# haoheliu/voicefixer

Measured on AMD Instinct MI355X. Metric: seconds-of-44.1kHz-audio restored per wall-second, higher is better.
Workload: dtype f32

## Files before the change

### voicefixer_amd/csrc/vfx_conv.hip

```cpp
#include "vfx_common.h"
#include <cstdio>
#include <cstdlib>
#include <cstring>
#include <map>
#include <mutex>
#include <string>
#include <type_traits>
#include <vector>

#ifndef VFX_X3_ABL
#define VFX_X3_ABL 0
#endif
#ifndef VFX_ABL
#define VFX_ABL 0
#endif
#define VFX_MAXPH 8
#define VFX_MAXT 9

typedef float f32x16 __attribute__((ext_vector_type(16)));
typedef unsigned int u32x4 __attribute__((ext_vector_type(4)));

#if VFX_ABL & 8
__device__ unsigned long long g_dbg[10];
__device__ unsigned long long g_dbgx[6];
extern "C" int vfx_debug_read(unsigned long long* out, int reset) {
    hipMemcpyFromSymbol(out, HIP_SYMBOL(g_dbg), sizeof(unsigned long long) * 10);
    if (reset) { unsigned long long z[10] = {0}; hipMemcpyToSymbol(HIP_SYMBOL(g_dbg), z, sizeof(z)); }
    return 0;
}
extern "C" int vfx_debug_read_x(unsigned long long* out, int reset) {
    hipMemcpyFromSymbol(out, HIP_SYMBOL(g_dbgx), sizeof(unsigned long long) * 6);
    if (reset) { unsigned long long z[6] = {0}; hipMemcpyToSymbol(HIP_SYMBOL(g_dbgx), z, sizeof(z)); }
    return 0;
}
__device__ unsigned long long* g_trace_buf;
__device__ unsigned int g_trace_cap, g_trace_n;
extern "C" int vfx_debug_trace(unsigned long long* buf, unsigned int cap_records) {
    const unsigned int z = 0;
    hipMemcpyToSymbol(HIP_SYMBOL(g_trace_buf), &buf, sizeof(buf));
    hipMemcpyToSymbol(HIP_SYMBOL(g_trace_cap), &cap_records, sizeof(cap_records));
    hipMemcpyToSymbol(HIP_SYMBOL(g_trace_n), &z, sizeof(z));
    return 0;
}
extern "C" unsigned int vfx_debug_trace_count(void) {
    unsigned int n = 0;
    hipMemcpyFromSymbol(&n, HIP_SYMBOL(g_trace_n), sizeof(n));
    return n;
}
#define DBG_T(v) const unsigned long long v = __builtin_amdgcn_s_memtime()
#else
#define DBG_T(v)
#endif

struct PhaseTab {
    int ntaps, nseg, ooff, pad_;
    int seg_org[VFX_MAXT];
    int tap_lds[VFX_MAXT];
    int tap_w[VFX_MAXT];
};
struct ConvTables {
    PhaseTab ph[VFX_MAXPH];
};

struct ConvArgs {
    const float* x;
    const float* w;
    const float* bias;
    const float* res;
    float* y;
    const float* pre_scale;
    const float* pre_shift;
    const ConvTables* tab;
    int B, Cin, CinPad, Cout, Lin, Lq, Lout;
    long long x_bs, x_cs, y_bs, y_cs, y_ls, r_bs, r_cs, r_ls;
    int segw;
    int xs_floats;
    int ws_floats;
    int q_shift, q_mask, o_rs, o_cs;
    int pad_mode, pre_act, post_act;
    float pre_slope, post_slope;
    int in_mask, out_mask;
    int tile_lo, tile_hi;
    int tpw;
    int x_guard;
    int ksplit, cpp, ws_ls;
    float* ws;
    int bl_step;
    int nxv;
    int two_level;
    int res_init;
    const void* w3;
    const ConvTables* tab3;
    int segw3;
    int xplane3;
    int buf3;
    int bl3;
    int xrow3, wrow3;
    const float* wd;
    int kcx;
    int ntiles_l, xcd_chunk;
    int nph_fold;
    int wg_d;
    const int* x_rows;
    int lq_extra;
    int stagger, stagger_wgs;
    int w_tap0, w_tapstep, w_slab0, w_slabstep, w_slab_ph, w_ooff0, w_ooff_ph, w_nseg, w_seg0, w_segstep;
    const float* wd2;
    const float* bias2;
    int yp;
    float mid_slope;
    int rb_nq1;
    int rs_pshift, rs_nseg;
};

template <int KC>
struct StageCfg {
    static constexpr int MAXXV = 4;
    static constexpr int MAXWV = KC == 16 ? 6 : (KC == 8 ? 4 : 5);
};

template <int MAXXV, int MAXWV>
struct StageState {
    int x_l[MAXXV];
    int x_kc[MAXXV];
    int x_off[MAXXV];
    int w_off[MAXWV];
    float4 xv[MAXXV];
    float4 wv[MAXWV];
};

template <bool FAST, int MAXXV, int MAXWV>
__device__ __forceinline__ void stage_load(StageState<MAXXV, MAXWV>& st, const ConvArgs& a,
                                           const float* __restrict__ xb, int xcs, int c0, int lshift,
                                           __amdgpu_buffer_rsrc_t xrsrc, __amdgpu_buffer_rsrc_t wrsrc, int Lin_row) {
    if constexpr (FAST) {
        const int xso = (c0 * xcs + lshift) * 4, wso = c0 * a.Cout * 4;
#pragma unroll
        for (int j = 0; j < MAXXV; ++j) {
            const u32x4 r = __builtin_amdgcn_raw_buffer_load_b128(xrsrc, st.x_off[j], xso, 0);
            st.xv[j] = make_float4(__uint_as_float(r.x), __uint_as_float(r.y), __uint_as_float(r.z), __uint_as_float(r.w));
        }
#pragma unroll
        for (int j = 0; j < MAXWV; ++j) {
            const u32x4 r = __builtin_amdgcn_raw_buffer_load_b128(wrsrc, st.w_off[j], wso, 0);
            st.wv[j] = make_float4(__uint_as_float(r.x), __uint_as_float(r.y), __uint_as_float(r.z), __uint_as_float(r.w));
        }
        return;
    }
    const float* __restrict__ xc = xb + (long long)c0 * xcs + lshift;
    const float* __restrict__ wc = a.w + (long long)c0 * a.Cout;
#pragma unroll
    for (int j = 0; j < MAXXV; ++j) {
        if constexpr (FAST) {
            st.xv[j] = *reinterpret_cast<const float4*>(xc + st.x_off[j]);
        } else {
            const int Lin = Lin_row;
            const bool reflect = a.pad_mode == VFX_PAD_REFLECT;
            float4 v = make_float4(0.f, 0.f, 0.f, 0.f);
            const int kc = st.x_kc[j];
            if (c0 + kc < a.Cin) {
                const float* row = xc + (long long)kc * xcs;
                const int l = st.x_l[j];
                if (l >= 0 && l + 3 < Lin) {
                    v = *reinterpret_cast<const float4*>(row + l);
                } else {
                    float e[4];
#pragma unroll
                    for (int k = 0; k < 4; ++k) {
                        int g = l + k;
                        if (reflect) {
                            if (g < 0) g = -g;
                            if (g >= Lin) g = 2 * (Lin - 1) - g;
                        }
                        e[k] = (g >= 0 && g < Lin) ? row[g] : 0.f;
                    }
                    v = make_float4(e[0], e[1], e[2], e[3]);
                }
            }
            st.xv[j] = v;
        }
    }
#pragma unroll
    for (int j = 0; j < MAXWV; ++j) st.wv[j] = *reinterpret_cast<const float4*>(wc + st.w_off[j]);
}

template <int NTHR, int MAXXV, int MAXWV>
__device__ __forceinline__ void stage_write_plain(StageState<MAXXV, MAXWV>& st, const ConvArgs& a, float* xs, float* ws,
                                                  int nxv, int nwv, int xtotal, int wtotal, int tid) {
    const float slope = a.pre_act == VFX_PRE_LRELU ? a.pre_slope : 1.f;
#pragma unroll
    for (int j = 0; j < MAXXV; ++j) {
        if (j < nxv) {
            float4 v = st.xv[j];
            v.x = v.x > 0.f ? v.x : v.x * slope;
            v.y = v.y > 0.f ? v.y : v.y * slope;
            v.z = v.z > 0.f ? v.z : v.z * slope;
            v.w = v.w > 0.f ? v.w : v.w * slope;
            int i = tid + NTHR * j;
            i = i < xtotal ? i : xtotal - 1;
            *reinterpret_cast<float4*>(xs + 4 * i) = v;
        }
    }
#pragma unroll
    for (int j = 0; j < MAXWV; ++j)
        if (j < nwv) {
            int i = tid + NTHR * j;
            i = i < wtotal ? i : wtotal - 1;
            *reinterpret_cast<float4*>(ws + 4 * i) = st.wv[j];
        }
}

template <bool FAST, int NTHR, int MAXXV, int MAXWV>
__device__ __forceinline__ void stage_write(StageState<MAXXV, MAXWV>& st, const ConvArgs& a, int c0, float* xs,
                                            float* ws, const float* aff, int nxv, int nwv, int xtotal,
                                            int wtotal, int tid, int lshift, bool range_mask, int Lin_row) {
    const int pre_act = a.pre_act;
    const float pre_slope = a.pre_slope;
    const int in_mask = a.in_mask;
#pragma unroll
    for (int j = 0; j < MAXXV; ++j) {
        if (j < nxv) {
            float e[4] = {st.xv[j].x, st.xv[j].y, st.xv[j].z, st.xv[j].w};
            if (pre_act == VFX_PRE_LRELU) {
#pragma unroll
                for (int k = 0; k < 4; ++k) e[k] = vfx_lrelu(e[k], pre_slope);
            } else if (pre_act == VFX_PRE_AFFINE_LRELU) {
                const int c = c0 + st.x_kc[j];
                const float sc = aff[2 * c], sh = aff[2 * c + 1];
#pragma unroll
                for (int k = 0; k < 4; ++k) e[k] = vfx_lrelu(fmaf(e[k], sc, sh), pre_slope);
                if constexpr (!FAST) {
                    const int l = st.x_l[j] + lshift;
                    const bool cbad = c >= a.Cin;
                    if (a.pad_mode != VFX_PAD_REFLECT) {
#pragma unroll
                        for (int k = 0; k < 4; ++k)
                            if (l + k < 0 || l + k >= Lin_row || cbad) e[k] = 0.f;
                    }
                }
            }
            if constexpr (FAST) {
                if (range_mask) {
                    const int l = st.x_l[j] + lshift;
#pragma unroll
                    for (int k = 0; k < 4; ++k)
                        if (l + k < 0 || l + k >= Lin_row) e[k] = 0.f;
                }
            }
            if (in_mask >= 3) {
                const int l = st.x_l[j] + lshift;
                if (((l + 3) & in_mask) == in_mask) e[3] = 0.f;
            } else if (in_mask) {
                const int l = st.x_l[j] + lshift;
#pragma unroll
                for (int k = 0; k < 4; ++k)
                    if (((l + k) & in_mask) == in_mask) e[k] = 0.f;
            }
            int i = tid + NTHR * j;
            i = i < xtotal ? i : xtotal - 1;
            *reinterpret_cast<float4*>(xs + 4 * i) = make_float4(e[0], e[1], e[2], e[3]);
        }
    }
#pragma unroll
    for (int j = 0; j < MAXWV; ++j)
        if (j < nwv) {
// ... 1081 lines not shown
        const float quant = (float)nwg / (float)(((nwg + slots - 1) / slots) * slots);
        const float score = t.util * tail * quant;
        if (score > best_score * 1.02f) { best_score = score; best = i; }
    }
    if (best < 0) return VFX_EINVAL;
    const TileCfg& tc = kTiles[best];

    static const bool waves8_env = VFX_DEV_ENV("VFX_WAVES8") && atoi(VFX_DEV_ENV("VFX_WAVES8")) != 0;
    const bool waves8 = waves8_env && ((tc.BM == 128 && tc.BL == 128) || (tc.BM == 64 && tc.BL == 256));
    const int nthr = waves8 ? 512 : 256;
    static const bool kc16_env = VFX_DEV_ENV("VFX_KC16") && atoi(VFX_DEV_ENV("VFX_KC16")) != 0;
    int maxspan = 0;
    bool all_segments = true;
    for (int p = 0; p < nphase; ++p) {
        int mn = phs[p].taps[0].off, mx = mn;
        for (int t = 1; t < phs[p].ntaps; ++t) {
            mn = phs[p].taps[t].off < mn ? phs[p].taps[t].off : mn;
            mx = phs[p].taps[t].off > mx ? phs[p].taps[t].off : mx;
        }
        maxspan = mx - mn > maxspan ? mx - mn : maxspan;
        all_segments &= !((long long)tc.BL + (mx - mn) + 3 <= (long long)phs[p].ntaps * (tc.BL + 3));
    }
    static const int exact_off = VFX_DEV_ENV("VFX_NO_EXACT") ? atoi(VFX_DEV_ENV("VFX_NO_EXACT")) : 0;
    bool exact = exact_off != 1 && x->guard > 0 && pad_mode != VFX_PAD_REFLECT && in_mask == 0 && !waves8 &&
                 ((maxspan > 0 && maxspan <= 8) || (all_segments && exact_off != 2));
    ConvTables tb;
    int KC, ntiles;
    size_t lds;
    for (;;) {
        KC = (kc16_env && maxnt <= 3 && tc.BM == 128 && tc.BL == 128 && !waves8 && Cin % 16 == 0) ? 16 : 8;
        for (;;) {
            std::memset(&tb, 0, sizeof(tb));
            int rc = fill_segments(a, tb, nphase, phs, tc.BL, KC, exact);
            if (rc) return rc;
            int maxseg = 0;
            for (int p = 0; p < nphase; ++p) maxseg = tb.ph[p].nseg > maxseg ? tb.ph[p].nseg : maxseg;
            const bool xfit = (long long)maxseg * KC * (a.segw / 4) <= 4 * nthr;
            a.nxv = (int)(((long long)maxseg * KC * (a.segw / 4) + nthr - 1) / nthr);
            const bool wfit = (long long)maxnt * KC * tc.BM <= (KC == 16 ? 6 : (KC == 8 ? 4 : 5)) * 4 * nthr;
            if (xfit && wfit) break;
            if (KC == 4) return VFX_ERANGE;
            KC = KC == 16 ? 8 : 4;
        }
        a.ws_floats = maxnt * KC * tc.BM;
        lds = (2ull * (a.xs_floats + a.ws_floats) + 2ull * a.CinPad) * sizeof(float);
        {
            static const long pad_kb = VFX_DEV_ENV("VFX_LDS_MIN_KB") ? atol(VFX_DEV_ENV("VFX_LDS_MIN_KB")) : 0;
            if (pad_kb > 0 && lds < (size_t)pad_kb * 1024) lds = (size_t)pad_kb * 1024;
        }
        if (lds > 160 * 1024) return VFX_ERANGE;

        a.bl_step = (exact && !all_segments) ? tc.BL - maxspan : tc.BL;
        ntiles = (Lq + a.bl_step - 1) / a.bl_step;
        int seg_lo = 0x7fffffff, seg_hi = -0x7fffffff;
        for (int p = 0; p < nphase; ++p)
            for (int sg = 0; sg < tb.ph[p].nseg; ++sg) {
                seg_lo = tb.ph[p].seg_org[sg] < seg_lo ? tb.ph[p].seg_org[sg] : seg_lo;
                seg_hi = tb.ph[p].seg_org[sg] > seg_hi ? tb.ph[p].seg_org[sg] : seg_hi;
            }
        const long long g = (x->guard > 0 && pad_mode != VFX_PAD_REFLECT) ? x->guard : 0;
        const long long need_lo = -(long long)seg_lo - g;
        int tlo = need_lo > 0 ? (int)((need_lo + a.bl_step - 1) / a.bl_step) : 0;
        const long long room = (long long)Lin + g - seg_hi - a.segw;
        int thi = room >= 0 ? (int)(room / a.bl_step) + 1 : 0;
        if (thi > ntiles) thi = ntiles;
        if (tlo > thi || Cin % KC != 0) { tlo = 0; thi = 0; }
        if (((long long)a.CinPad * x->cstride + Lin + 2 * g) * 4 >= (1ll << 31) - (1ll << 20)) { tlo = 0; thi = 0; }
        if (a.x_rows && pad_mode == VFX_PAD_REFLECT) { tlo = 0; thi = 0; }
        a.tile_lo = tlo;
        a.tile_hi = thi;
        if (exact && !(tlo == 0 && thi == ntiles)) { exact = false; continue; }
        break;
    }
    a.tab = device_tables(tb);
    if (!a.tab) return VFX_EINVAL;
    a.two_level = KC == 4 && Cin >= 256;
    g_last_tile = tc.BM * 100000 + tc.BL * 100 + KC;
    a.ksplit = 1;
    {
        static const bool splitk_off = VFX_DEV_ENV("VFX_NO_SPLITK") && atoi(VFX_DEV_ENV("VFX_NO_SPLITK")) != 0;
        const int nchunks = (Cin + KC - 1) / KC;
        const long long nwg = (long long)ntiles * (nphase * Cout / tc.BM) * B;
        const bool plain_map = nphase == 1 && q_shift == 31 && o_rs == 0 && o_cs == 1 && phs[0].ooff == 0 && Lq <= Lout;
        if (!splitk_off && plain_map && nwg <= 192 && nchunks >= 32) {
            int want = (int)(512 / nwg);
            if (want > 8) want = 8;
            if (want > nchunks / 16) want = nchunks / 16;
            if (want >= 2 && (long long)B * want <= 65535) {
                a.cpp = (nchunks + want - 1) / want;
                a.ksplit = (nchunks + a.cpp - 1) / a.cpp;
                a.ws_ls = Lq;
                a.ws = splitk_workspace(stream, (size_t)a.ksplit * B * Cout * Lq * sizeof(float));
                if (!a.ws) a.ksplit = 1;
            }
        }
    }
    {
        const long long nwg1 = (long long)(a.tile_hi - a.tile_lo) * (nphase * Cout / tc.BM) * B;
        (void)nwg1;
        a.tpw = 1;
    }
    const int gy = nphase * Cout / tc.BM;
    const int gz = B * a.ksplit;
    int rc = VFX_EINVAL;
    if (KC == 16) rc = launch_cfg<128, 128, 2, 2, 16>(a, ntiles, gy, gz, lds, stream);
#define VFX_CASE(BM_, BL_, WGM_, WGL_)                                                          \
    else if (tc.BM == BM_ && tc.BL == BL_)                                                      \
        rc = KC == 8 ? launch_cfg<BM_, BL_, WGM_, WGL_, 8>(a, ntiles, gy, gz, lds, stream)      \
                     : launch_cfg<BM_, BL_, WGM_, WGL_, 4>(a, ntiles, gy, gz, lds, stream);
    else if (waves8 && tc.BM == 128 && tc.BL == 128)
        rc = KC == 8 ? launch_cfg<128, 128, 4, 2, 8>(a, ntiles, gy, gz, lds, stream)
                     : launch_cfg<128, 128, 4, 2, 4>(a, ntiles, gy, gz, lds, stream);
    else if (waves8 && tc.BM == 64 && tc.BL == 256)
        rc = KC == 8 ? launch_cfg<64, 256, 2, 4, 8>(a, ntiles, gy, gz, lds, stream)
                     : launch_cfg<64, 256, 2, 4, 4>(a, ntiles, gy, gz, lds, stream);
    VFX_CASE(128, 128, 2, 2)
    VFX_CASE(64, 256, 1, 4)
    VFX_CASE(128, 64, 4, 1)
    VFX_CASE(32, 256, 1, 4)
    VFX_CASE(64, 64, 2, 2)
    VFX_CASE(32, 128, 1, 4)
#undef VFX_CASE
    if (rc != VFX_OK || a.ksplit == 1) return rc;
    const long long total = (long long)B * Cout * Lq;
    const int blocks = (int)((total + 255) / 256 < 4096 ? (total + 255) / 256 : 4096);
    hipLaunchKernelGGL(splitk_reduce_kernel, dim3(blocks), dim3(256), 0, stream, a.ws, a.ksplit, a.ws_ls, a.bias, a.res,
                       a.r_bs, a.r_cs, a.r_ls, a.y, a.y_bs, a.y_cs, a.y_ls, B, Cout, Lq, a.post_act, a.post_slope,
                       a.out_mask);
    VFX_LAUNCHED();
    return vfx_last_error();
}

extern "C" int vfx_conv1d_f32(const vfx_tensor* x, const float* w_packed, const float* bias,
                              const vfx_tensor* res, const vfx_tensor* y, int B, int Cin, int Cout,
                              int L, int k, int dilation, int pad_mode, const vfx_act* act,
                              vfx_stream_t stream) {
    if (k < 1 || k > VFX_MAXT || !(k & 1) || dilation < 1) return VFX_EINVAL;
    PhaseSpec ph;
    ph.ntaps = k;
    ph.ooff = 0;
    for (int t = 0; t < k; ++t) {
        ph.taps[t].off = (t - (k - 1) / 2) * dilation;
        ph.taps[t].slab = t;
    }
    return launch_conv(x, w_packed, bias, res, y, B, Cin, Cout, L, L, L, 1, &ph, 31, 0x7fffffff, 0, 1,
                       pad_mode, act, 0, 0, (hipStream_t)stream);
}

extern "C" int vfx_convtr1d_f32(const vfx_tensor* x, const float* w_packed, const float* bias,
                                const vfx_tensor* y, int B, int Cin, int Cout, int Lin, int stride,
                                const vfx_act* act, vfx_stream_t stream) {
    if (stride < 1 || stride > VFX_MAXPH) return VFX_EINVAL;
    if (act && act->w_wino4) {
        const int rc = try_launch_convtw(x, act->w_wino4, bias, y, B, Cin, Cout, Lin, stride, act, (hipStream_t)stream);
        if (rc != VFX_ENOTSUP) return rc;
    }
    const int pad = stride / 2 + stride % 2;
    PhaseSpec ph[VFX_MAXPH];
    for (int r = 0; r < stride; ++r) {
        ph[r].ntaps = 2;
        ph[r].taps[0].off = 0;
        ph[r].taps[0].slab = r;
        ph[r].taps[1].off = -1;
        ph[r].taps[1].slab = r + stride;
        ph[r].ooff = r - pad;
    }
    return launch_conv(x, w_packed, bias, nullptr, y, B, Cin, Cout, Lin, Lin + 1, stride * Lin, stride, ph,
                       31, 0x7fffffff, 0, stride, VFX_PAD_ZERO, act, 0, 0, (hipStream_t)stream);
}

extern "C" int vfx_conv2d_f32(const vfx_tensor* x, const float* w_packed, const float* bias,
                              const vfx_tensor* res, const vfx_tensor* y, int B, int Cin, int Cout, int H,
                              int pitch_log2, int ksize, const vfx_act* act, vfx_stream_t stream) {
    if ((ksize != 1 && ksize != 3) || pitch_log2 < 1 || pitch_log2 > 12 || H < 1) return VFX_EINVAL;
    const int P = 1 << pitch_log2;
    PhaseSpec ph;
    ph.ooff = 0;
    ph.ntaps = ksize * ksize;
    for (int ky = 0; ky < ksize; ++ky)
        for (int kx = 0; kx < ksize; ++kx) {
            ph.taps[ky * ksize + kx].off = (ky - ksize / 2) * P + (kx - ksize / 2);
            ph.taps[ky * ksize + kx].slab = ky * ksize + kx;
        }
    const int L = H * P;
    return launch_conv(x, w_packed, bias, res, y, B, Cin, Cout, L, L, L, 1, &ph, 31, 0x7fffffff, 0, 1,
                       VFX_PAD_ZERO, act, P - 1, P - 1, (hipStream_t)stream);
}

extern "C" int vfx_convtr2d_3x3s2_f32(const vfx_tensor* x, const float* w_packed, const vfx_tensor* y, int B,
                                      int Cin, int Cout, int h, int in_pitch_log2, const vfx_act* act,
                                      vfx_stream_t stream) {
    if (in_pitch_log2 < 1 || in_pitch_log2 > 11 || h < 1) return VFX_EINVAL;
    const int Pi = 1 << in_pitch_log2, Po = 2 * Pi;
    PhaseSpec ph[4];
    for (int py = 0; py < 2; ++py)
        for (int px = 0; px < 2; ++px) {
            PhaseSpec& p = ph[py * 2 + px];
            p.ntaps = 0;
            p.ooff = py * Po + px;
            const int nky = py == 0 ? 2 : 1, nkx = px == 0 ? 2 : 1;
            for (int iy = 0; iy < nky; ++iy)
                for (int ix = 0; ix < nkx; ++ix) {
                    const int ky = py == 0 ? 2 * iy : 1, kx = px == 0 ? 2 * ix : 1;
                    const int dy = py == 0 ? iy : 0, dx = px == 0 ? ix : 0;
                    p.taps[p.ntaps].off = -(dy * Pi + dx);
                    p.taps[p.ntaps].slab = ky * 3 + kx;
                    ++p.ntaps;
                }
        }
    const int Lin = h * Pi;
    return launch_conv(x, w_packed, nullptr, nullptr, y, B, Cin, Cout, Lin, Lin, 2 * h * Po, 4, ph,
                       in_pitch_log2, Pi - 1, 2 * Po, 2, VFX_PAD_ZERO, act, Pi - 1, Po - 1,
                       (hipStream_t)stream);
}
```

### voicefixer_amd/csrc/vfx_convtw.inc

```
template <int WGM, int WGP>
__global__ __launch_bounds__(256, 2) void convtw_kernel(const ConvArgs a) {
    static_assert(WGM * WGP == 4, "four waves");
    constexpr int KC = 16, NSTEP = KC / 2, NPL = 4;
    constexpr int BM = 32 * WGM, BT = 32 * WGP;
    constexpr int CG = 256 / BT;
    constexpr int NSLOT = KC / CG;
    constexpr int SPAN = NSTEP / NSLOT;
    constexpr int PLANE = KC * BT;
    constexpr int BUF = NPL * PLANE;
    extern __shared__ __attribute__((aligned(16))) float smem[];

    const int tid = threadIdx.x, lane = tid & 63;
    const int wave = __builtin_amdgcn_readfirstlane(tid >> 6);
    const int lo = lane & 31, hi = lane >> 5;
    const int wm = wave / WGP, wp = wave % WGP;
    const int s = a.nph_fold, gy = a.tpw;
    int lin = blockIdx.x;
    if (a.xcd_chunk > 0) lin = (lin & 7) * a.xcd_chunk + (lin >> 3);
    if (lin >= a.ntiles_l * s * gy) return;
    int phase, mblk, tile;
    if (a.tile_lo == 0) {
        tile = lin % a.ntiles_l;
        const int rest = lin / a.ntiles_l;
        phase = rest % s; mblk = rest / s;
    } else {
        phase = lin % s;
        const int rest = lin / s;
        mblk = rest % gy; tile = rest / gy;
    }
    const int b = blockIdx.z;
    const int Lrow = a.x_rows ? __builtin_amdgcn_readfirstlane(a.x_rows[b]) : a.Lin;
    const int T0 = tile * BT;
    if (3 * T0 > Lrow) return;
    const int xcs = (int)a.x_cs;
    const int S = a.Cin / KC;

    const int st = tid % BT, cg = tid / BT;
    int xvoff[4];
    {
        const int p0 = 3 * (T0 + st) - 1;
#pragma unroll
        for (int j = 0; j < 4; ++j) xvoff[j] = (p0 + j >= 0 && p0 + j < Lrow) ? (cg * xcs + p0 + j) * 4 : VFX_W_OOB;
    }
    const __amdgpu_buffer_rsrc_t xrsrc = __builtin_amdgcn_make_buffer_rsrc(
        const_cast<float*>(a.x) + (long long)b * a.x_bs, (short)0, 0x7fffffff, 0x00020000);
    float* const wbase = smem + cg * BT + st;
    float xv[NSLOT][4];
    auto x_load_part = [&](int j, int t, int s0) {
        xv[j][t] = __uint_as_float(__builtin_amdgcn_raw_buffer_load_b32(xrsrc, xvoff[t], s0 + j * CG * xcs * 4, 0));
    };
    auto x_load = [&](int chunk) {
        const int s0 = chunk * KC * xcs * 4;
#pragma unroll
        for (int j = 0; j < NSLOT; ++j)
#pragma unroll
            for (int t = 0; t < 4; ++t) x_load_part(j, t, s0);
    };
    auto x_transform = [&](int j, float (&V)[4]) {
        V[0] = xv[j][0] - xv[j][2];
        V[1] = xv[j][1] + xv[j][2];
        V[2] = xv[j][2] - xv[j][1];
        V[3] = xv[j][3] - xv[j][1];
    };

    const __amdgpu_buffer_rsrc_t wrsrc =
        __builtin_amdgcn_make_buffer_rsrc(const_cast<float*>(a.wd), (short)0, 0x7fffffff, 0x00020000);
    const int row0 = mblk * BM + wm * 32;
    const int avoff = ((row0 + lo) * 8 + 4 * hi) * 4;
    const int gstride = a.Cout * 32;
    const int pstride = (a.CinPad >> 3) * gstride;
    const int poff = phase * NPL * pstride;
    float4 aw[2][NPL];
    auto a_load_one = [&](auto set_tag, int k, int grp) {
        constexpr int SET = decltype(set_tag)::value;
        const u32x4 r = __builtin_amdgcn_raw_buffer_load_b128(wrsrc, avoff, poff + k * pstride + grp * gstride, 0);
        aw[SET][k] = make_float4(__uint_as_float(r.x), __uint_as_float(r.y), __uint_as_float(r.z), __uint_as_float(r.w));
    };
    using S0 = std::integral_constant<int, 0>;
    using S1 = std::integral_constant<int, 1>;

    const __amdgpu_buffer_rsrc_t brsrc = __builtin_amdgcn_make_buffer_rsrc(
        const_cast<float*>(a.bias ? a.bias : a.x), (short)0, 0x7fffffff, 0x00020000);
    u32x4 bq[4];
    {
        const int bvoff = a.bias ? (row0 + 4 * hi) * 4 : VFX_W_OOB;
#pragma unroll
        for (int g = 0; g < 4; ++g) bq[g] = __builtin_amdgcn_raw_buffer_load_b128(brsrc, bvoff, g * 32, 0);
    }
    x_load(0);
#pragma unroll
    for (int k = 0; k < NPL; ++k) a_load_one(S0{}, k, 0);
    __builtin_amdgcn_sched_barrier(0);

    f32x16 acc[NPL];
    const int boffs = hi * BT + wp * 32 + lo;
    f32x16 biasv;
#pragma unroll
    for (int g = 0; g < 4; ++g) {
        biasv[4 * g + 0] = __uint_as_float(bq[g].x); biasv[4 * g + 1] = __uint_as_float(bq[g].y);
        biasv[4 * g + 2] = __uint_as_float(bq[g].z); biasv[4 * g + 3] = __uint_as_float(bq[g].w);
    }
    auto mma_chunk = [&](auto first_tag, const float* xs, float* wdst, int xchunk, int agrp0) {
        constexpr bool FIRST = decltype(first_tag)::value;
        const float* bp = xs + boffs;
        const int agrp1 = min(agrp0 + 1, 2 * S - 1), agrp2 = min(agrp0 + 2, 2 * S - 1);
        float bf[NPL];
#pragma unroll
        for (int k = 0; k < NPL; ++k) bf[k] = bp[k * PLANE];
        const int xs0 = xchunk * KC * xcs * 4;
        float V[4];
#pragma unroll
        for (int u = 0; u < NSTEP; ++u) {
            const int el = u / SPAN, ph = u % SPAN;
#pragma unroll
            for (int k = 0; k < NPL; ++k) {
                if (ph == 0 && k == 0) x_transform(el, V);
                if (ph == 0) wdst[el * CG * BT + k * PLANE] = V[k];
                if (ph == SPAN / 2) x_load_part(el, k, xs0);
                if (u == 0) a_load_one(S1{}, k, agrp1);
                if (u == 4) a_load_one(S0{}, k, agrp2);
                const float4 av4 = (u < 4) ? aw[0][k] : aw[1][k];
                const int kk = u & 3;
                const float av = kk == 0 ? av4.x : (kk == 1 ? av4.y : (kk == 2 ? av4.z : av4.w));
                if (FIRST && u == 0) {
                    const f32x16 zero16 = {0.f, 0.f, 0.f, 0.f, 0.f, 0.f, 0.f, 0.f, 0.f, 0.f, 0.f, 0.f, 0.f, 0.f, 0.f, 0.f};
                    acc[k] = __builtin_amdgcn_mfma_f32_32x32x2f32(av, bf[k], k == 1 ? biasv : zero16, 0, 0, 0);
                } else {
                    acc[k] = __builtin_amdgcn_mfma_f32_32x32x2f32(av, bf[k], acc[k], 0, 0, 0);
                }
                if (u < NSTEP - 1) bf[k] = bp[k * PLANE + (u + 1) * 2 * BT];
                __builtin_amdgcn_sched_barrier(0);
            }
        }
    };
    {
#pragma unroll
        for (int j = 0; j < NSLOT; ++j) {
            float V[4];
            x_transform(j, V);
#pragma unroll
            for (int k = 0; k < NPL; ++k) wbase[j * CG * BT + k * PLANE] = V[k];
        }
        x_load(1);
        __builtin_amdgcn_sched_barrier(0);
    }
    __syncthreads();
    mma_chunk(std::true_type{}, smem, wbase + BUF, 2 < S ? 2 : S - 1, 0);
    __syncthreads();
    mma_chunk(std::false_type{}, smem + BUF, wbase, 3 < S ? 3 : S - 1, 2);
    __syncthreads();
#pragma unroll 1
    for (int c = 2; c < S; c += 2) {
        mma_chunk(std::false_type{}, smem, wbase + BUF, min(c + 2, S - 1), 2 * c);
        __syncthreads();
        mma_chunk(std::false_type{}, smem + BUF, wbase, min(c + 3, S - 1), 2 * c + 2);
        __syncthreads();
    }

    const __amdgpu_buffer_rsrc_t yrsrc = __builtin_amdgcn_make_buffer_rsrc(
        a.y + (long long)b * a.y_bs, (short)0, 0x7fffffff, 0x00020000);
    const int ycs4 = (int)a.y_cs * 4;
    const int q0 = 3 * (T0 + wp * 32 + lo);
    int yv[3];
#pragma unroll
    for (int i = 0; i < 3; ++i) {
        const int q = q0 + i;
        const int o = q * s + phase - a.w_ooff0;
        yv[i] = (q <= Lrow && o >= 0 && o < s * Lrow) ? (4 * hi * (int)a.y_cs + o) * 4 : VFX_W_OOB;
    }
#pragma unroll
    for (int r = 0; r < 16; ++r) {
        const int soff = (row0 + (r & 3) + 8 * (r >> 2)) * ycs4;
        const float p12 = acc[1][r] + acc[2][r];
        const float y0 = acc[0][r] + p12;
        const float y1 = acc[1][r] - acc[2][r];
        const float y2 = p12 + acc[3][r];
        __builtin_amdgcn_raw_buffer_store_b32(__float_as_uint(y0), yrsrc, yv[0], soff, 0);
        __builtin_amdgcn_raw_buffer_store_b32(__float_as_uint(y1), yrsrc, yv[1], soff, 0);
        __builtin_amdgcn_raw_buffer_store_b32(__float_as_uint(y2), yrsrc, yv[2], soff, 0);
    }
}

template <int WGM, int WGP>
static int launch_convtw(const ConvArgs& a, dim3 grid, size_t lds, hipStream_t s) {
    hipLaunchKernelGGL((convtw_kernel<WGM, WGP>), grid, dim3(256), lds, s, a);
    VFX_LAUNCHED();
    return vfx_last_error();
}

static int try_launch_convtw(const vfx_tensor* x, const float* w32, const float* bias, const vfx_tensor* y, int B, int Cin, int Cout,
                             int Lin, int stride, const vfx_act* act, hipStream_t stream) {
    static const bool off = VFX_DEV_ENV("VFX_CONVTW") && atoi(VFX_DEV_ENV("VFX_CONVTW")) == 0;
    if (off || !w32 || !vfx_aligned16(w32) || !x || !y || !x->ptr || !y->ptr) return VFX_ENOTSUP;
    if (act && (act->pre_act != VFX_PRE_NONE || act->post_act != VFX_POST_NONE || act->math != VFX_MATH_F32)) return VFX_ENOTSUP;
    if (Cin % 32 != 0 || Cout % 64 != 0 || B <= 0 || B > 65535 || Lin < 1 || stride < 1) return VFX_ENOTSUP;
    if (x->lstride != 1 || y->lstride != 1 || (bias && !vfx_aligned16(bias))) return VFX_ENOTSUP;
    const long long lim = (1ll << 31) - (1ll << 20);
    if (((long long)Cin * x->cstride + Lin) * 4 >= lim || ((long long)Cout * y->cstride + (long long)stride * Lin) * 4 >= lim) return VFX_ENOTSUP;
    if (4ll * stride * (Cin >> 3) * Cout * 32 >= lim) return VFX_ENOTSUP;
    const bool wide = Cout % 128 == 0;
    const int BT = wide ? 32 : 64;
    const int ntriples = (Lin + 1 + 2) / 3;
    const int ntiles = (ntriples + BT - 1) / BT;
    const int gy = Cout / (wide ? 128 : 64);
    const long long nwg = (long long)ntiles * stride * gy;
    if (nwg * B < 512 || nwg >= (1ll << 30)) return VFX_ENOTSUP;
    ConvArgs a;
    std::memset(&a, 0, sizeof(a));
    a.x = (const float*)x->ptr;
    a.wd = w32;
    a.bias = bias;
    a.y = (float*)y->ptr;
    a.B = B; a.Cin = Cin; a.CinPad = Cin; a.Cout = Cout;
    a.Lin = Lin; a.Lq = Lin + 1; a.Lout = stride * Lin;
    a.x_bs = x->bstride; a.x_cs = x->cstride;
    a.x_rows = x->rows;
    a.y_bs = y->bstride; a.y_cs = y->cstride; a.y_ls = 1;
    a.nph_fold = stride;
    a.tpw = gy;
    a.w_ooff0 = stride / 2 + stride % 2;
    a.ntiles_l = ntiles;
    a.tile_lo = 16ll * stride * Cin * Cout <= (3ll << 20) ? 1 : 0;
    if (VFX_DEV_ENV("VFX_CONVTW_ORDER")) a.tile_lo = atoi(VFX_DEV_ENV("VFX_CONVTW_ORDER")) == 0 ? 1 : 0;
    a.xcd_chunk = nwg >= 64 ? (int)((nwg + 7) / 8) : 0;
    const dim3 grid(a.xcd_chunk > 0 ? (unsigned)(8 * a.xcd_chunk) : (unsigned)nwg, 1, B);
    const size_t lds = 2ull * 4 * 16 * BT * sizeof(float);
    g_last_tile = (wide ? 128 : 64) * 100000 + 3 * BT * 100 + 83;
    return wide ? launch_convtw<4, 1>(a, grid, lds, stream) : launch_convtw<2, 2>(a, grid, lds, stream);
}
```

### voicefixer_amd/packing.py

```python
import torch


def _pad_cin(w):
    cin = w.shape[1]
    cpad = (cin + 7) // 8 * 8
    if cpad != cin:
        w = torch.cat([w, w.new_zeros(w.shape[0], cpad - cin, w.shape[2])], dim=1)
    return w.contiguous().float()


def pack_conv1d(w):
    return _pad_cin(w.permute(2, 1, 0))


def pack_convtr1d(w):
    return _pad_cin(w.permute(2, 0, 1))


def pack_conv2d(w):
    co, ci, kh, kw = w.shape
    return _pad_cin(w.permute(2, 3, 1, 0).reshape(kh * kw, ci, co))


def pack_convtr2d(w):
    ci, co, kh, kw = w.shape
    return _pad_cin(w.permute(2, 3, 0, 1).reshape(kh * kw, ci, co))


def pack_linear(w):
    return _pad_cin(w.t()[None])


def pack_direct(w_packed):
    s, cp, co = w_packed.shape
    assert cp % 8 == 0
    w = w_packed.reshape(s, cp // 8, 8, co)[:, :, [0, 2, 4, 6, 1, 3, 5, 7], :]
    return w.permute(0, 1, 3, 2).contiguous().float()


def pack_wino(w_packed):
    assert w_packed.shape[0] == 3
    g = w_packed.double()
    u = torch.stack([g[0], (g[0] + g[1] + g[2]) * 0.5, (g[0] - g[1] + g[2]) * 0.5, g[2]])
    return pack_direct(u.float())


def pack_wino4(w_packed):
    assert w_packed.shape[0] == 3
    g0, g1, g2 = w_packed.double()
    u = torch.stack([g0 / 4, -(g0 + g1 + g2) / 6, -(g0 - g1 + g2) / 6, g0 / 24 + g1 / 12 + g2 / 6,
                     g0 / 24 - g1 / 12 + g2 / 6, g2])
    return pack_direct(u.float())


def pack_wino32_tr(w_packed, stride):
    assert w_packed.shape[0] == 2 * stride
    g = w_packed.double()
    planes = []
    for r in range(stride):
        g0, g1 = g[r + stride], g[r]
        planes += [g0, (g0 + g1) * 0.5, (g0 - g1) * 0.5, g1]
    return pack_direct(torch.stack(planes).float())


def _f43(g0, g1, g2):
    return [g0 / 4, -(g0 + g1 + g2) / 6, -(g0 - g1 + g2) / 6, g0 / 24 + g1 / 12 + g2 / 6, g0 / 24 - g1 / 12 + g2 / 6, g2]


def pack_wino4_2d(w_packed):
    assert w_packed.shape[0] == 9
    g = w_packed.double().reshape(3, 3, w_packed.shape[1], w_packed.shape[2])
    planes = []
    for kx in range(3):
        planes += _f43(g[0, kx], g[1, kx], g[2, kx])
    return pack_direct(torch.stack(planes).float())


def pack_cout1(w):
    return w.reshape(w.shape[1], -1).contiguous().float()


def pack_gru_whh(w_hh_fwd, w_hh_bwd, kreg, klds, kstr):
    assert kreg + klds + kstr == 128 and kstr % 4 == 0
    out = []
    for w in (w_hh_fwd, w_hh_bwd):
        wt = w.float().t().contiguous()
        wt = wt.reshape(2, 128, 768)
        r = wt[:, :kreg].reshape(-1)
        l = wt[:, kreg:kreg + klds].reshape(-1)
        st = wt[:, kreg + klds:].reshape(2, kstr // 4, 4, 3, 256)
        st = st.permute(0, 1, 3, 4, 2).reshape(-1)
        out.append(torch.cat([r, l, st]))
    return torch.cat(out).contiguous()


def pack_x3(w_packed):
    s, cin, cout = w_packed.shape
    if cout % 32 != 0:
        return None
    c16 = (cin + 15) // 16 * 16
    w = w_packed.float()
    if c16 != cin:
        w = torch.cat([w, w.new_zeros(s, c16 - cin, cout)], dim=1)
    hi = w.to(torch.bfloat16)
    lo = (w - hi.float()).to(torch.bfloat16)
    planes = torch.stack([hi, lo], dim=1)
    planes = planes.reshape(s, 2, c16 // 16, 2, 8, cout)
    return planes.permute(0, 2, 1, 3, 5, 4).contiguous()


F16_MAX = 65504.0


def pack_f16(w_packed):
    s, cin, cout = w_packed.shape
    if s != 3 or cin != cout or cout not in (128, 256, 512):
        return None
    w = w_packed.float()
    if not bool(torch.isfinite(w).all()) or float(w.abs().max()) > F16_MAX:
        return None
    w = w.reshape(3, cin // 8, 8, cout).permute(0, 1, 3, 2)
    return w.to(torch.float16).contiguous()
```

Before: 1635.

## Fold transposed-conv phases into output rows and stage stores through LDS

The Winograd transposed-conv kernel stops launching one workgroup per phase. The weights are repacked so that the stride phases are interleaved into the Cout dimension, which makes each output row of the GEMM map to a (channel, phase) pair, computed with a magic-number division. The epilogue stages interior results in per-wave LDS so it can issue contiguous 128-bit global stores instead of strided scalar stores, and it keeps scalar stores only for the partial channels at block edges. This adds division arithmetic, more LDS use and wave-level barriers, and it needs the unpacked weight pointer for validation.

```diff
diff --git a/voicefixer_amd/csrc/vfx_conv.hip b/voicefixer_amd/csrc/vfx_conv.hip
--- a/voicefixer_amd/csrc/vfx_conv.hip
+++ b/voicefixer_amd/csrc/vfx_conv.hip
@@ -111,6 +111,7 @@
     float mid_slope;
     int rb_nq1;
     int rs_pshift, rs_nseg;
+    unsigned tw_rdiv;
 };
 
 template <int KC>
@@ -1498,7 +1499,7 @@
                                 const vfx_act* act, vfx_stream_t stream) {
     if (stride < 1 || stride > VFX_MAXPH) return VFX_EINVAL;
     if (act && act->w_wino4) {
-        const int rc = try_launch_convtw(x, act->w_wino4, bias, y, B, Cin, Cout, Lin, stride, act, (hipStream_t)stream);
+        const int rc = try_launch_convtw(x, w_packed, act->w_wino4, bias, y, B, Cin, Cout, Lin, stride, act, (hipStream_t)stream);
         if (rc != VFX_ENOTSUP) return rc;
     }
     const int pad = stride / 2 + stride % 2;
diff --git a/voicefixer_amd/csrc/vfx_convtw.inc b/voicefixer_amd/csrc/vfx_convtw.inc
--- a/voicefixer_amd/csrc/vfx_convtw.inc
+++ b/voicefixer_amd/csrc/vfx_convtw.inc
@@ -17,16 +17,12 @@
     const int s = a.nph_fold, gy = a.tpw;
     int lin = blockIdx.x;
     if (a.xcd_chunk > 0) lin = (lin & 7) * a.xcd_chunk + (lin >> 3);
-    if (lin >= a.ntiles_l * s * gy) return;
-    int phase, mblk, tile;
+    if (lin >= a.ntiles_l * gy) return;
+    int mblk, tile;
     if (a.tile_lo == 0) {
-        tile = lin % a.ntiles_l;
-        const int rest = lin / a.ntiles_l;
-        phase = rest % s; mblk = rest / s;
+        tile = lin % a.ntiles_l; mblk = lin / a.ntiles_l;
     } else {
-        phase = lin % s;
-        const int rest = lin / s;
-        mblk = rest % gy; tile = rest / gy;
+        mblk = lin % gy; tile = lin / gy;
     }
     const int b = blockIdx.z;
     const int Lrow = a.x_rows ? __builtin_amdgcn_readfirstlane(a.x_rows[b]) : a.Lin;
@@ -67,25 +63,35 @@
         __builtin_amdgcn_make_buffer_rsrc(const_cast<float*>(a.wd), (short)0, 0x7fffffff, 0x00020000);
     const int row0 = mblk * BM + wm * 32;
     const int avoff = ((row0 + lo) * 8 + 4 * hi) * 4;
-    const int gstride = a.Cout * 32;
+    const int gstride = s * a.Cout * 32;
     const int pstride = (a.CinPad >> 3) * gstride;
-    const int poff = phase * NPL * pstride;
     float4 aw[2][NPL];
     auto a_load_one = [&](auto set_tag, int k, int grp) {
         constexpr int SET = decltype(set_tag)::value;
-        const u32x4 r = __builtin_amdgcn_raw_buffer_load_b128(wrsrc, avoff, poff + k * pstride + grp * gstride, 0);
+        const u32x4 r = __builtin_amdgcn_raw_buffer_load_b128(wrsrc, avoff, k * pstride + grp * gstride, 0);
         aw[SET][k] = make_float4(__uint_as_float(r.x), __uint_as_float(r.y), __uint_as_float(r.z), __uint_as_float(r.w));
     };
     using S0 = std::integral_constant<int, 0>;
     using S1 = std::integral_constant<int, 1>;
 
+    const int s1mask = s == 1 ? -1 : 0;
+    auto row_cp = [&](int R, int& c, int& p) {
+        c = (int)__umulhi((unsigned)R, a.tw_rdiv) + (R & s1mask);
+        p = R - c * s;
+    };
     const __amdgpu_buffer_rsrc_t brsrc = __builtin_amdgcn_make_buffer_rsrc(
         const_cast<float*>(a.bias ? a.bias : a.x), (short)0, 0x7fffffff, 0x00020000);
-    u32x4 bq[4];
+    unsigned bq[16];
     {
-        const int bvoff = a.bias ? (row0 + 4 * hi) * 4 : VFX_W_OOB;
-#pragma unroll
-        for (int g = 0; g < 4; ++g) bq[g] = __builtin_amdgcn_raw_buffer_load_b128(brsrc, bvoff, g * 32, 0);
+#pragma unroll
+        for (int r = 0; r < 16; ++r) {
+            const int k = (r & 3) + 8 * (r >> 2);
+            int c0, p0, c1, p1;
+            row_cp(row0 + k, c0, p0);
+            row_cp(row0 + k + 4, c1, p1);
+            const int bvoff = a.bias ? (hi ? c1 : c0) * 4 : VFX_W_OOB;
+            bq[r] = __builtin_amdgcn_raw_buffer_load_b32(brsrc, bvoff, 0, 0);
+        }
     }
     x_load(0);
 #pragma unroll
@@ -96,10 +102,7 @@
     const int boffs = hi * BT + wp * 32 + lo;
     f32x16 biasv;
 #pragma unroll
-    for (int g = 0; g < 4; ++g) {
-        biasv[4 * g + 0] = __uint_as_float(bq[g].x); biasv[4 * g + 1] = __uint_as_float(bq[g].y);
-        biasv[4 * g + 2] = __uint_as_float(bq[g].z); biasv[4 * g + 3] = __uint_as_float(bq[g].w);
-    }
+    for (int r = 0; r < 16; ++r) biasv[r] = __uint_as_float(bq[r]);
     auto mma_chunk = [&](auto first_tag, const float* xs, float* wdst, int xchunk, int agrp0) {
         constexpr bool FIRST = decltype(first_tag)::value;
         const float* bp = xs + boffs;
@@ -159,25 +162,88 @@
 
     const __amdgpu_buffer_rsrc_t yrsrc = __builtin_amdgcn_make_buffer_rsrc(
         a.y + (long long)b * a.y_bs, (short)0, 0x7fffffff, 0x00020000);
-    const int ycs4 = (int)a.y_cs * 4;
+    const int ycs = (int)a.y_cs, pad = a.w_ooff0;
     const int q0 = 3 * (T0 + wp * 32 + lo);
-    int yv[3];
-#pragma unroll
-    for (int i = 0; i < 3; ++i) {
-        const int q = q0 + i;
-        const int o = q * s + phase - a.w_ooff0;
-        yv[i] = (q <= Lrow && o >= 0 && o < s * Lrow) ? (4 * hi * (int)a.y_cs + o) * 4 : VFX_W_OOB;
-    }
+    const int qs4[3] = {q0 * s * 4, (q0 + 1) * s * 4, (q0 + 2) * s * 4};
+    int rowe = row0;
+    asm volatile("" : "+s"(rowe));
+    const bool edge = __any(q0 == 0 || q0 + 2 >= Lrow);
+    constexpr int HT = 16;
+    float* const lt = smem + wave * (32 * 3 * HT);
+    int cA, pA, nfull, rem;
+    row_cp(rowe, cA, pA);
+    const int jf = pA == 0 ? 0 : s - pA;
+    const int cf = pA == 0 ? cA : cA + 1;
+    row_cp(32 - jf, nfull, rem);
+    const int jt = 32 - rem;
+    const int cspan = 3 * HT * s, sL = s * Lrow;
 #pragma unroll
     for (int r = 0; r < 16; ++r) {
-        const int soff = (row0 + (r & 3) + 8 * (r >> 2)) * ycs4;
-        const float p12 = acc[1][r] + acc[2][r];
-        const float y0 = acc[0][r] + p12;
-        const float y1 = acc[1][r] - acc[2][r];
-        const float y2 = p12 + acc[3][r];
-        __builtin_amdgcn_raw_buffer_store_b32(__float_as_uint(y0), yrsrc, yv[0], soff, 0);
-        __builtin_amdgcn_raw_buffer_store_b32(__float_as_uint(y1), yrsrc, yv[1], soff, 0);
-        __builtin_amdgcn_raw_buffer_store_b32(__float_as_uint(y2), yrsrc, yv[2], soff, 0);
+        const int k = (r & 3) + 8 * (r >> 2);
+        const bool part0 = k < jf || k >= jt, part1 = k + 4 < jf || k + 4 >= jt;
+        if (part0 || part1) {
+            int c0, p0, c1, p1;
+            row_cp(rowe + k, c0, p0);
+            row_cp(rowe + k + 4, c1, p1);
+            const float p12 = acc[1][r] + acc[2][r];
+            const float yo[3] = {acc[0][r] + p12, acc[1][r] - acc[2][r], p12 + acc[3][r]};
+            const int rowb = hi ? (c1 * ycs + p1 - pad) * 4 : (c0 * ycs + p0 - pad) * 4;
+            const int o0 = hi ? p1 - pad : p0 - pad;
+            const bool mine = hi ? part1 : part0;
+#pragma unroll
+            for (int i = 0; i < 3; ++i) {
+                const int o = (q0 + i) * s + o0;
+                const int yv = (mine && o >= 0 && o < sL) ? rowb + qs4[i] : VFX_W_OOB;
+                __builtin_amdgcn_raw_buffer_store_b32(__float_as_uint(yo[i]), yrsrc, yv, 0, 0);
+            }
+        }
+    }
+    const int nv = nfull * (cspan >> 2);
+    const float inv_cv = 1.0f / (float)(cspan >> 2);
+#pragma unroll
+    for (int h = 0; h < 2; ++h) {
+        const int tl = lo - HT * h;
+        if (tl >= 0 && tl < HT) {
+#pragma unroll
+            for (int r = 0; r < 16; ++r) {
+                const int k = (r & 3) + 8 * (r >> 2);
+                int c0, p0, c1, p1;
+                row_cp(rowe + k, c0, p0);
+                row_cp(rowe + k + 4, c1, p1);
+                const bool whole = hi ? (k + 4 >= jf && k + 4 < jt) : (k >= jf && k < jt);
+                if (whole) {
+                    const float p12 = acc[1][r] + acc[2][r];
+                    float* const d = lt + (hi ? (c1 - cf) * cspan + p1 : (c0 - cf) * cspan + p0) + 3 * tl * s;
+                    d[0] = acc[0][r] + p12;
+                    d[s] = acc[1][r] - acc[2][r];
+                    d[2 * s] = p12 + acc[3][r];
+                }
+            }
+        }
+        __builtin_amdgcn_fence(__ATOMIC_ACQ_REL, "wavefront");
+        __builtin_amdgcn_wave_barrier();
+        const int os = 3 * (T0 + wp * 32 + HT * h) * s - pad;
+        for (int v = lane; v < nv; v += 64) {
+            const int cl = fast_div(v, cspan >> 2, inv_cv);
+            const int w4 = (v - cl * (cspan >> 2)) * 4;
+            const float4 d = *reinterpret_cast<const float4*>(lt + cl * cspan + w4);
+            const u32x4 u = {__float_as_uint(d.x), __float_as_uint(d.y), __float_as_uint(d.z), __float_as_uint(d.w)};
+            const int o4 = os + w4;
+            const int yb = ((cf + cl) * ycs + o4) * 4;
+            if (!edge) {
+                __builtin_amdgcn_raw_buffer_store_b128(u, yrsrc, yb, 0, 0);
+            } else {
+                const bool all4 = o4 >= 0 && o4 + 3 < sL;
+                __builtin_amdgcn_raw_buffer_store_b128(u, yrsrc, all4 ? yb : VFX_W_OOB, 0, 0);
+#pragma unroll
+                for (int j = 0; j < 4; ++j) {
+                    const bool one = !all4 && o4 + j >= 0 && o4 + j < sL;
+                    __builtin_amdgcn_raw_buffer_store_b32(u[j], yrsrc, one ? yb + 4 * j : VFX_W_OOB, 0, 0);
+                }
+            }
+        }
+        __builtin_amdgcn_fence(__ATOMIC_ACQ_REL, "wavefront");
+        __builtin_amdgcn_wave_barrier();
     }
 }
 
@@ -188,16 +254,16 @@
     return vfx_last_error();
 }
 
-static int try_launch_convtw(const vfx_tensor* x, const float* w32, const float* bias, const vfx_tensor* y, int B, int Cin, int Cout,
-                             int Lin, int stride, const vfx_act* act, hipStream_t stream) {
+static int try_launch_convtw(const vfx_tensor* x, const float* w_packed, const float* w32, const float* bias, const vfx_tensor* y, int B,
+                             int Cin, int Cout, int Lin, int stride, const vfx_act* act, hipStream_t stream) {
     static const bool off = VFX_DEV_ENV("VFX_CONVTW") && atoi(VFX_DEV_ENV("VFX_CONVTW")) == 0;
-    if (off || !w32 || !vfx_aligned16(w32) || !x || !y || !x->ptr || !y->ptr) return VFX_ENOTSUP;
+    if (off || !w_packed || !w32 || !vfx_aligned16(w32) || !x || !y || !x->ptr || !y->ptr) return VFX_ENOTSUP;
     if (act && (act->pre_act != VFX_PRE_NONE || act->post_act != VFX_POST_NONE || act->math != VFX_MATH_F32)) return VFX_ENOTSUP;
-    if (Cin % 32 != 0 || Cout % 64 != 0 || B <= 0 || B > 65535 || Lin < 1 || stride < 1) return VFX_ENOTSUP;
+    if (Cin < 32 || Cout <= 0 || Cin % 32 != 0 || Cout % 64 != 0 || B <= 0 || B > 65535 || Lin < 1 || stride < 1) return VFX_ENOTSUP;
     if (x->lstride != 1 || y->lstride != 1 || (bias && !vfx_aligned16(bias))) return VFX_ENOTSUP;
     const long long lim = (1ll << 31) - (1ll << 20);
     if (((long long)Cin * x->cstride + Lin) * 4 >= lim || ((long long)Cout * y->cstride + (long long)stride * Lin) * 4 >= lim) return VFX_ENOTSUP;
-    if (4ll * stride * (Cin >> 3) * Cout * 32 >= lim) return VFX_ENOTSUP;
+    if (4ll * stride * (Cin >> 3) * Cout * 32 >= lim || (long long)stride * stride * Cout >= (1ll << 32)) return VFX_ENOTSUP;
     const bool wide = Cout % 128 == 0;
     const int BT = wide ? 32 : 64;
     const int ntriples = (Lin + 1 + 2) / 3;
@@ -217,14 +283,15 @@
     a.x_rows = x->rows;
     a.y_bs = y->bstride; a.y_cs = y->cstride; a.y_ls = 1;
     a.nph_fold = stride;
-    a.tpw = gy;
+    a.tpw = stride * gy;
     a.w_ooff0 = stride / 2 + stride % 2;
+    a.tw_rdiv = (unsigned)(((1ull << 32) + stride - 1) / stride);
     a.ntiles_l = ntiles;
     a.tile_lo = 16ll * stride * Cin * Cout <= (3ll << 20) ? 1 : 0;
     if (VFX_DEV_ENV("VFX_CONVTW_ORDER")) a.tile_lo = atoi(VFX_DEV_ENV("VFX_CONVTW_ORDER")) == 0 ? 1 : 0;
     a.xcd_chunk = nwg >= 64 ? (int)((nwg + 7) / 8) : 0;
     const dim3 grid(a.xcd_chunk > 0 ? (unsigned)(8 * a.xcd_chunk) : (unsigned)nwg, 1, B);
-    const size_t lds = 2ull * 4 * 16 * BT * sizeof(float);
+    const size_t lds = (wide ? 4ull * 32 * 48 : 2ull * 4 * 16 * BT) * sizeof(float);
     g_last_tile = (wide ? 128 : 64) * 100000 + 3 * BT * 100 + 83;
     return wide ? launch_convtw<4, 1>(a, grid, lds, stream) : launch_convtw<2, 2>(a, grid, lds, stream);
 }
diff --git a/voicefixer_amd/packing.py b/voicefixer_amd/packing.py
--- a/voicefixer_amd/packing.py
+++ b/voicefixer_amd/packing.py
@@ -56,11 +56,10 @@
 def pack_wino32_tr(w_packed, stride):
     assert w_packed.shape[0] == 2 * stride
     g = w_packed.double()
-    planes = []
-    for r in range(stride):
-        g0, g1 = g[r + stride], g[r]
-        planes += [g0, (g0 + g1) * 0.5, (g0 - g1) * 0.5, g1]
-    return pack_direct(torch.stack(planes).float())
+    g0, g1 = g[stride:], g[:stride]
+    u = torch.stack([g0, (g0 + g1) * 0.5, (g0 - g1) * 0.5, g1])
+    cp, co = w_packed.shape[1:]
+    return pack_direct(u.permute(0, 2, 3, 1).reshape(4, cp, co * stride).float())
 
 
 def _f43(g0, g1, g2):
```

After: 1653 (median of 6 runs). +1.1%, better.
